# google-deepmind/meltingpot

Hardware: AMD Instinct MI355X
Metric: agent-steps/sec (env_batch x players / wall s), clean_up @4096 worlds (higher is better)
Workload: dtype u8

## Files before the change

### include/mp_engine.h

```cpp
#ifndef MP_ENGINE_H_
#define MP_ENGINE_H_

#include <stdint.h>

#ifdef __cplusplus
extern "C" {
#endif
#pragma GCC visibility push(default)

#define MP_ABI_VERSION 8

enum {
  MP_OK = 0,
  MP_ERR_INVALID = -1,
  MP_ERR_PACK = -2,
  MP_ERR_NO_DEVICE = -3,
  MP_ERR_HIP = -4,
  MP_ERR_UNSUPPORTED = -5
};

typedef enum {
  MP_EVENT_ZAP = 1,
  MP_EVENT_EDIBLE_CONSUMED = 2,
  MP_EVENT_PLAYER_CLEANED = 3,
// ... 47 lines not shown

typedef struct MpEngine MpEngine;

typedef struct {
  uint32_t struct_size;
  int32_t batch_worlds;
  int32_t waves;
  int32_t feeders;
  int32_t max_groups;
  int32_t scratch_cells;
  int32_t no_composite_cache;
  int32_t max_composites;
  int32_t verbose;
  int32_t late_feeder_prio;
  int32_t ring_batches;
  int32_t static_pct;
  int32_t world_waves;
  int32_t store_sc1;
  int32_t head;
  int32_t no_next_orders;
  int32_t record_pad;
  int32_t pace;
  int32_t team;
} MpDevOptions;

typedef struct {
  uint32_t struct_size;
  int32_t device;
  int32_t num_worlds;
  int32_t auto_reset;
  uint64_t world_offset;
  uint64_t base_seed;
  void* stream;
  int32_t num_players;
  int32_t debug_observations;
  int32_t unfused;
  int32_t literal_base_seed;
  const MpDevOptions* dev;
  const int32_t* roles;
  int32_t world_pool;
} MpConfig;

typedef struct {
  int32_t abi_version;
  int32_t substrate;
  int32_t num_worlds, num_players, num_actions;
// ... 4 lines not shown
  int32_t fused;
  int32_t num_resources;
  int32_t num_action_fields;
  int32_t plan_batch_worlds, plan_ring_batches, plan_owned_batches, plan_pooled_batches,
          plan_groups, plan_store_sc1 ;
  int32_t plan_feeders, plan_waves;
  int32_t ring_slots, ring_next;
  int32_t plan_pace, visible_layers;
  int32_t plan_team, plan_late_priority;
  int64_t retired_va_bytes, retired_va_limit;
} MpInfo;

int mp_abi_version(void);

const char* mp_last_error(void);

int mp_create(const void* pack, uint64_t pack_len, const MpConfig* cfg,
              MpEngine** out);

void mp_destroy(MpEngine* eng);

int mp_info(const MpEngine* eng, MpInfo* out);

int mp_set_stream(MpEngine* eng, void* stream);

int mp_bind_output(MpEngine* eng, MpObsKind kind, void* device_ptr);

int mp_bind_output_ring(MpEngine* eng, MpObsKind kind, void* base,
                        uint64_t slot_stride_bytes, int32_t slots);

int mp_reset(MpEngine* eng, const uint64_t* seeds, const uint8_t* mask);

int mp_step(MpEngine* eng, const int32_t* actions_device);

int mp_step_host(MpEngine* eng, const int32_t* actions_host);

int mp_step_fields(MpEngine* eng, const int32_t* fields_device);

int mp_step_fields_host(MpEngine* eng, const int32_t* fields_host);

int mp_observe(MpEngine* eng, MpObsKind kind, void* dst_device);

uint64_t mp_obs_bytes(const MpEngine* eng, MpObsKind kind);

int mp_dump(MpEngine* eng, uint8_t* grid, int32_t* avat, int32_t* glob);

// ... 76 lines not shown
```

### meltingpot_amd/_build.py

```python

from __future__ import annotations

import fcntl
import os
import shutil
import subprocess

_HERE = os.path.dirname(os.path.abspath(__file__))
CSRC = os.path.join(_HERE, "csrc")
LIB_DIR = os.path.join(_HERE, "lib")
LIB_PATH = os.path.join(LIB_DIR, "libmp_engine.so")
SOURCES = ("mp_engine.hip", "pack_decode.hip", "step_kernels.hip", "step_many.hip", "frame.hip", "frame_wpool2.hip",
           "frame_wpool4.hip", "frame_wpool8.hip")
HEADERS = ("mp_common.h", "pack_decode.h", "frame_kernel.h", "frame_wpool.h", "step_common.h", "step_clean_up.h", "step_commons.h",
           "step_territory.h", "step_coins.h", "step_matrix.h", "step_coop.h", "step_gift.h", "step_cook.h", "step_mushroom.h", "step_load.h", "../../include/mp_engine.h",
           "../../include/mp_pack.h", "exports.map")
ARCH = "gfx950"


def _stale() -> bool:
  if not os.path.exists(LIB_PATH):
    return True
  built = os.path.getmtime(LIB_PATH)
  for f in SOURCES + HEADERS:
    if os.path.getmtime(os.path.join(CSRC, f)) > built:
      return True
  return False


def build_engine(force: bool = False, verbose: bool = False) -> str:
  if not force and not _stale():
    return LIB_PATH
  hipcc = shutil.which("hipcc") or "/opt/rocm/bin/hipcc"
  if not os.path.exists(hipcc):
    raise RuntimeError("hipcc not found: cannot build libmp_engine.so")
  os.makedirs(LIB_DIR, exist_ok=True)
  with open(os.path.join(LIB_DIR, ".build.lock"), "w") as lock:
# ... 41 lines not shown
```

### meltingpot_amd/csrc/frame.hip

```cpp
#include "frame_kernel.h"

static int slot_scratch_bytes(const DevTables& t, const SubstrateTables& s) {
  int extra = 0;
  if (s.substrate == MPK_SUBSTRATE_TERRITORY) extra = stepk::extra_bytes(s.tr);
  if (s.substrate == MPK_SUBSTRATE_EXTERNALITY_MUSHROOMS) extra = stepk::extra_bytes(s.em);
  return stepk::scratch_bytes(t) + extra;
}


FramePlan plan_frame(const DevTables& t, const SubstrateTables& s, int num_worlds,
                     bool with_step, int views, int num_cus, const MpDevOptions* dev, int pool_k,
                     int world_k) {
  FramePlan p = {};
  const int lds_pool = pool_k > 1 && views != 1 ? pool_k : 0;
  const int lds_wpool = world_k > 1 && views != 0 ? world_k : 0;
  const bool world_view = views == 1;
  const int max_waves = ((with_step && s.substrate == MPK_SUBSTRATE_THE_MATRIX) ? kMatrixThreads
                                                                                : kDrawThreads) / 64;
  p.nwaves = world_view ? 12 : 16;
  p.feeders = 4;
  int B = 4, NB = 2;
  if (with_step && !world_view && max_waves == 16) {
    B = 3;
    p.feeders = s.substrate == MPK_SUBSTRATE_THE_MATRIX ? 6
// ... 217 lines not shown

template <class Tables, class Sites>
int allow_lds() {
  const void* k[9] = {
      reinterpret_cast<const void*>(&k_frame<Tables, Sites, 0>),
      reinterpret_cast<const void*>(&k_frame<Tables, Sites, 1>),
      reinterpret_cast<const void*>(&k_frame<Tables, Sites, 2>),
      reinterpret_cast<const void*>(&k_frame<Tables, Sites, 0, 2>),
      reinterpret_cast<const void*>(&k_frame<Tables, Sites, 2, 2>),
      reinterpret_cast<const void*>(&k_frame<Tables, Sites, 0, 4>),
      reinterpret_cast<const void*>(&k_frame<Tables, Sites, 2, 4>),
      reinterpret_cast<const void*>(&k_frame<Tables, Sites, 0, 8>),
      reinterpret_cast<const void*>(&k_frame<Tables, Sites, 2, 8>)};
  hipError_t r[9];
  for (int i = 0; i < 9; ++i)
    r[i] = hipFuncSetAttribute(k[i], hipFuncAttributeMaxDynamicSharedMemorySize, 160 * 1024);
  for (hipError_t e : r)
    if (e != hipSuccess) return (int)e;
  return 0;
}

}

int prepare_frame() {
  int rc = prepare_frame_wpool<2>();
  if (!rc) rc = prepare_frame_wpool<4>();
  if (!rc) rc = prepare_frame_wpool<8>();
  if (!rc) rc = allow_lds<NoTables, NoSites>();
  if (!rc) rc = allow_lds<CleanUpTables, stepk::CleanUpSites>();
#if !defined(MP_FRAME_ISA_SUBSET)
  if (!rc) rc = allow_lds<CommonsTables, stepk::CommonsSites>();
  if (!rc) rc = allow_lds<TerritoryTables, stepk::TerritorySites>();
  if (!rc) rc = allow_lds<CoinsTables, stepk::CoinsSites>();
  if (!rc) rc = allow_lds<MatrixTables, stepk::MatrixSites>();
  if (!rc) rc = allow_lds<CoopTables, stepk::CoopSites>();
  if (!rc) rc = allow_lds<GiftTables, stepk::GiftSites>();
  if (!rc) rc = allow_lds<CookTables, stepk::CookSites>();
  if (!rc) rc = allow_lds<MushroomTables, stepk::MushroomSites>();
#endif
  return rc;
}

void launch_frame(const DevTables& t, const SubstrateTables* s, const stepk::StepArgs& args,
                  uint8_t* out_a, uint8_t* out_w, const FramePlan& p, hipStream_t stream, int pool_k,
                  int world_k) {
  if (out_w && world_k > 1) {
    if (world_k == 2) launch_frame_wpool<2>(t, s, args, out_a, out_w, p, stream, pool_k);
    else if (world_k == 4) launch_frame_wpool<4>(t, s, args, out_a, out_w, p, stream, pool_k);
    else launch_frame_wpool<8>(t, s, args, out_a, out_w, p, stream, pool_k);
    return;
  }
  if (!s) {
    launch_one<NoTables, NoSites>(t, NoTables(), args, out_a, out_w, p, stream, pool_k);
    return;
  }
#if defined(MP_FRAME_ISA_SUBSET)
  if (s->substrate == MPK_SUBSTRATE_CLEAN_UP)
    launch_one<CleanUpTables, stepk::CleanUpSites>(t, s->cu, args, out_a, out_w, p, stream, pool_k);
#else
  switch (s->substrate) {
    case MPK_SUBSTRATE_CLEAN_UP:
      launch_one<CleanUpTables, stepk::CleanUpSites>(t, s->cu, args, out_a, out_w, p, stream, pool_k);
      break;
    case MPK_SUBSTRATE_COMMONS_HARVEST:
      launch_one<CommonsTables, stepk::CommonsSites>(t, s->ch, args, out_a, out_w, p, stream, pool_k);
      break;
    case MPK_SUBSTRATE_TERRITORY:
      launch_one<TerritoryTables, stepk::TerritorySites>(t, s->tr, args, out_a, out_w, p, stream, pool_k);
      break;
    case MPK_SUBSTRATE_COINS:
      launch_one<CoinsTables, stepk::CoinsSites>(t, s->co, args, out_a, out_w, p, stream, pool_k);
      break;
    case MPK_SUBSTRATE_THE_MATRIX:
      launch_one<MatrixTables, stepk::MatrixSites>(t, s->mx, args, out_a, out_w, p, stream, pool_k);
      break;
    case MPK_SUBSTRATE_COOP_MINING:
      launch_one<CoopTables, stepk::CoopSites>(t, s->cm, args, out_a, out_w, p, stream, pool_k);
      break;
// ... 13 lines not shown
```

### meltingpot_amd/csrc/frame_kernel.h

```cpp
#pragma once
#include <stdlib.h>
#include <string.h>

#include <type_traits>

#include "../../include/mp_pack.h"
#include "step_clean_up.h"
#include "step_coins.h"
#include "step_commons.h"
#include "step_coop.h"
#include "step_gift.h"
#include "step_mushroom.h"
#include "step_cook.h"
#include "step_matrix.h"
#include "step_territory.h"
#include "step_load.h"

template <bool kStep> constexpr bool nt_stores() { return kStep; }

namespace {

constexpr int kMaxLayers = 12;
constexpr int kSpriteStride = 272;
constexpr int kHeadBytes = 64;
// ... 321 lines not shown
constexpr uint64_t kMaxWaitTicks = 200000000ull;
enum { FAULT_BUFFER_FREE = 1, FAULT_BATCH_READY = 2, FAULT_PROLOGUE = 3, FAULT_CLAIM = 4 };
__device__ inline bool waited_too_long(uint32_t polls, uint64_t& t0) {
  if ((polls & 255u) != 255u) return false;
  const uint64_t now = wall_clock64();
  if (t0 == 0) { t0 = now; return false; }
  return now - t0 > kMaxWaitTicks;
}
__device__ inline void report_stall(const DevTables& t, int lane, uint32_t site, uint32_t wave,
                                    uint32_t batch, uint32_t seen, uint32_t wanted) {
  (void)lane;
  if (atomicCAS(&t.fault[0], 0u, site) == 0u) {
    t.fault[1] = blockIdx.x; t.fault[2] = wave; t.fault[3] = batch;
    t.fault[4] = seen; t.fault[5] = wanted;
  }
}

template <int kPool, int kWPool>
__device__ inline int pool_scratch_bytes(const DevTables& t) {
  if constexpr (kWPool == 0) return wave_scratch_bytes(t, kPool);
  else return wave_scratch_bytes(t, kPool, kWPool);
}

template <class Tables, class Sites, int kViews, int kPool = 0, int kWPool = 0>
__global__ __launch_bounds__(max_threads<Tables>()) void k_frame(DevTables t, Tables c,
                                                       stepk::StepArgs args,
                                                       uint8_t* __restrict__ out_a,
                                                       uint8_t* __restrict__ out_w,
                                                       FrameConsts K) {
  constexpr bool kStep = !std::is_same<Tables, NoTables>::value;
  constexpr bool kNt = nt_stores<kStep>();
#if defined(MP_FRAME_TIMELINE)
  const uint64_t tl_entry = wall_clock64();
#endif
  {
    constexpr int kArgBytes = (int)(sizeof(DevTables) + sizeof(Tables) + sizeof(stepk::StepArgs) +
                                    2 * sizeof(uint8_t*) + sizeof(FrameConsts));
    typedef const uint32_t __attribute__((address_space(4))) KernargWord;
    KernargWord* ka = (KernargWord*)__builtin_amdgcn_kernarg_segment_ptr();
    uint32_t warm = 0;
#pragma unroll
    for (int i = 0; i < kArgBytes / 4; i += 16) warm ^= ka[i];
    asm volatile("" ::"s"(warm));
  }
  extern __shared__ __attribute__((aligned(16))) uint8_t smem[];
  const FramePlan plan = K.p;
  const FrameLds lo = K.lo;
  const struct { int32_t N, nbt, chains, pool_first, b_mod_f, tables_vec, record_vec;
                 uint32_t first_k0, first_k1, magic_p, npb_all; } kc = {
      K.N, K.nbt, K.chains, K.pool_first, K.b_mod_f, K.tables_vec, K.record_vec,
      K.first_k_nibbles[0], K.first_k_nibbles[1], K.magic_p, K.npb_all};
  const int kWaves = plan.nwaves;
  const int B = plan.B, NB = plan.NB;
  const int F = plan.feeders;
// ... 995 lines not shown
```

### meltingpot_amd/csrc/mp_common.h

```cpp
#ifndef MP_COMMON_H_
#define MP_COMMON_H_

#include <hip/hip_runtime.h>
#include <stdint.h>

#include "../../include/mp_engine.h"

#define MP_MAX_PLAYERS 16
#define MP_WAVE 64

struct WorldTail {
  uint8_t ax[MP_MAX_PLAYERS];
  uint8_t ay[MP_MAX_PLAYERS];
  uint8_t aori[MP_MAX_PLAYERS];
  uint8_t aalive[MP_MAX_PLAYERS];
  uint8_t ztimer[MP_MAX_PLAYERS];
  uint8_t ctimer[MP_MAX_PLAYERS];
  uint8_t flag0[MP_MAX_PLAYERS];
  uint8_t flag1[MP_MAX_PLAYERS];
  uint8_t freeze[MP_MAX_PLAYERS];
  uint8_t removal[MP_MAX_PLAYERS];
  uint8_t aflags[MP_MAX_PLAYERS];
  uint8_t nozap[MP_MAX_PLAYERS];
  uint8_t level[MP_MAX_PLAYERS];
// ... 226 lines not shown
  int32_t n_site;
  const int32_t* site_cells;
  const int32_t* site_class;
  const int32_t* player_i32;
  const double* player_f64;
  int32_t R;
  int32_t res_layer, mark_layer, beam_layer, s_beam, hit;
  int32_t plane_a, plane_b;
  int32_t player_block;
  uint32_t s_visible_packed;
  uint64_t s_mark_packed;
  int32_t cooldown, respawn_frames, freeze, end_on_first, reset_winner, reset_loser,
      loser_dies, winner_dies, zero_inventory, random_tie, disallow_unready, has_ee,
      ee_min_frames, ee_interval, regen_delay, initial_health, n_intervals, spawn_all;
  double reward_floor, reward_multiplier, reward_unready;
  double row_matrix[9], col_matrix[9];
  double interval[10];
  uint64_t thr_regen, thr_ee;
  BeamShape shape;
};

struct SubstrateTables {
  int32_t substrate;
  CleanUpTables cu;
  CommonsTables ch;
  TerritoryTables tr;
  CoinsTables co;
  MatrixTables mx;
  CoopTables cm;
  GiftTables gr;
  CookTables cc;
  MushroomTables em;
};

struct StepOutputs {
  double* reward;
  double* ready;
  double* aux0;
  int32_t* step_type;
  double* discount;
  double* collective;
  int32_t* position;
  int32_t* orientation;
  int32_t* events;
  double* dbg[4];
  double* zap_matrix;
// ... 58 lines not shown
```

### meltingpot_amd/csrc/mp_engine.hip

```cpp
#include <chrono>
#include <map>
#include <mutex>
#include "../../include/mp_engine.h"

#include <stdarg.h>
#include <stddef.h>
#include <sys/types.h>
#include <stdio.h>
#include <string.h>

#include <algorithm>
#include <string>
#include <vector>

#include "pack_decode.h"
#include "step_common.h"

void launch_step(const DevTables& t, const SubstrateTables& s, const stepk::StepArgs& args,
                 hipStream_t stream);
void launch_step_many(const DevTables& t, const SubstrateTables& s, const stepk::StepArgs& args,
                      int steps, long long actions_step, void* const rows[5],
                      const uint64_t row_bytes[5], hipStream_t stream);
int step_lds_bytes(const DevTables& t, const SubstrateTables& s, int wpg);
int step_worlds_per_group(const DevTables& t, const SubstrateTables& s);
int prepare_step();
int prepare_step_many();
void launch_layer_view(const DevTables& t, const uint8_t* state, int32_t* out, int num_worlds,
                       hipStream_t stream);

constexpr int kFaultWords = 64 + 4 * 16 * 64 * 2;
FramePlan plan_frame(const DevTables& t, const SubstrateTables& s, int num_worlds,
                     bool with_step, int views, int num_cus, const MpDevOptions* dev,
                     int pool_k = 1,
                     int world_k = 1);
int frame_lds_bytes(const DevTables& t, const FramePlan& p, int pool_k = 1, int world_k = 1,
                    int views = 2);
int render_blob_bytes(const DevTables& t);
int prepare_frame();
// ... 719 lines not shown
    fprintf(stderr, "mp_engine: composite cache: %d images, %d table entries, probe %d\n",
            a.n_composites, a.used_slots, a.pair_probe);
  return MP_OK;
}

int upload_layer_lut(MpEngine* e) {
  const DevTables& t = e->t;
  const void* hp = e->pack.data();
  const int32_t* ssprite = table<int32_t>(hp, "state_sprite");
  const int32_t* vmap = table<int32_t>(hp, "view_sprite_map");
  std::vector<int32_t> lut((size_t)t.P * kLayerLutRow, 0);
  for (int p = 0; p < t.P; ++p) {
    const int32_t* remap = vmap + (size_t)p * t.nsprites;
    int32_t* row = lut.data() + (size_t)p * kLayerLutRow;
    for (int s = 1; s < t.nstates && s < 256; ++s)
      row[s] = ssprite[s] >= 0 ? 1 + remap[ssprite[s]] : 0;
    row[256] = 1 + remap[0];
  }
  HIP_TRY(hipMalloc((void**)&e->d_layer_lut, lut.size() * 4));
  HIP_TRY(hipMemcpy(e->d_layer_lut, lut.data(), lut.size() * 4, hipMemcpyHostToDevice));
  return MP_OK;
}

int plan_views(MpEngine* e, const MpDevOptions* dev) {
  const DevTables& t = e->t;
  for (int v = 0; v < 6; ++v) {
    FramePlan& pl = e->plan[v & 1][v >> 1];
    pl = plan_frame(t, e->sub, e->N, (v & 1) != 0, v >> 1, e->num_cus, dev);
    if (frame_lds_bytes(t, pl) > 160 * 1024)
      return fail(MP_ERR_PACK, "mp_create: renderer needs %d B of LDS", frame_lds_bytes(t, pl));
  }
  if (e->world_pool > 1)
    for (int v = 2; v < 6; ++v) {
      FramePlan& pl = e->plan[v & 1][v >> 1];
      pl = plan_frame(t, e->sub, e->N, (v & 1) != 0, v >> 1, e->num_cus, dev, 1, e->world_pool);
      const int need = frame_lds_bytes(t, pl, 1, e->world_pool, v >> 1);
      if (need > 160 * 1024)
        return fail(MP_ERR_UNSUPPORTED, "mp_create: WORLD.RGB pooled by %d (MpConfig.world_pool) needs "
                    "%d B of LDS", e->world_pool, need);
    }
  for (int i = 0; i < 3; ++i) {
    const int k = 2 << i;
    e->pool_ok[i] = t.sprite_size == 8;
    for (int v = 0; v < 6 && e->pool_ok[i]; ++v) {
      if ((v >> 1) == 1) continue;
      FramePlan& pl = e->pool_plan[i][v & 1][v >> 1];
// ... 18 lines not shown
              (v >> 1) == 0 ? "agents view" : (v >> 1) == 1 ? "world view" : "both views",
              pl.NB, pl.B, pl.feeders, pl.nwaves, pl.world_waves, pl.groups, pl.ks, pl.pool,
              frame_lds_bytes(t, pl, 1, e->world_pool, v >> 1));
    }
  return MP_OK;
}

int create_on_device(MpEngine* e, const MpConfig& cfg, DecodedPack* d) {
  const MpDevOptions* dev = cfg.dev;
  e->has_dev = dev != nullptr;
  e->next_orders = !(dev && dev->no_next_orders);
  e->device = cfg.device;
  e->N = cfg.num_worlds;
  e->auto_reset = cfg.auto_reset;
  e->stream = (hipStream_t)cfg.stream;
  e->unfused = cfg.unfused;
  e->world_pool = cfg.world_pool > 1 ? cfg.world_pool : 1;
  int cus = 0;
  if (hipDeviceGetAttribute(&cus, hipDeviceAttributeMultiprocessorCount, cfg.device) != hipSuccess ||
      cus <= 0)
    return fail(MP_ERR_NO_DEVICE, "mp_create: device %d does not report its compute units", cfg.device);
  e->num_cus = cus;
  int rc;
  if ((rc = upload_pack(e, cfg, d)) || (rc = alloc_fault_words(e)) || (rc = init_state(e, cfg)) ||
      (rc = alloc_outputs(e, cfg)) || (rc = build_atlas(e, dev, *d)) || (rc = upload_layer_lut(e)))
    return rc;
  return plan_views(e, dev);
}

}

extern "C" {

int mp_abi_version(void) { return MP_ABI_VERSION; }

const char* mp_last_error(void) { return g_error.c_str(); }

uint64_t mp_obs_bytes(const MpEngine* e, MpObsKind kind) {
  if (!e) return 0;
  const uint64_t N = (uint64_t)e->N, P = (uint64_t)e->t.P, S = (uint64_t)e->t.sprite_size;
  switch (kind) {
    case MP_OBS_RGB:
      return N * P * (e->t.vf + e->t.vb + 1) * S * (e->t.vl + e->t.vr + 1) * S * 3;
    case MP_OBS_WORLD_RGB: {
      const uint64_t k = (uint64_t)e->world_pool;
      return N * (e->t.H * S / k) * (e->t.W * S / k) * 3;
    }
    case MP_OBS_RGB_POOL2: case MP_OBS_RGB_POOL4: case MP_OBS_RGB_POOL8: {
      const uint64_t k = (uint64_t)MpEngine::pool_of(kind);
      if (!e->pool_ok[MpEngine::pool_index((int)k)]) return 0;
// ... 8 lines not shown
    case MP_OBS_AUX1: case MP_OBS_AUX2: case MP_OBS_AUX3: case MP_OBS_AUX4:
      return e->substrate == MPK_SUBSTRATE_CLEAN_UP ? N * P * 8 : 0;
    case MP_OBS_ZAP_MATRIX:
      return (e->substrate == MPK_SUBSTRATE_CLEAN_UP ||
              e->substrate == MPK_SUBSTRATE_COMMONS_HARVEST) ? N * P * P * 8 : 0;
    case MP_OBS_LAYER:
      return N * P * (e->t.vf + e->t.vb + 1) * (e->t.vl + e->t.vr + 1) * e->t.L * 4;
    case MP_OBS_INVENTORY:
      return N * P * e->inventory_types() * 8;
    case MP_OBS_INTERACTION_INVENTORIES:
      return e->substrate == MPK_SUBSTRATE_THE_MATRIX ? N * P * 2 * e->sub.mx.R * 8 : 0;
    case MP_OBS_MATRIX_CUMULANTS:
      return e->substrate == MPK_SUBSTRATE_THE_MATRIX ? N * P * (1 + 3 * e->sub.mx.R) * 8 : 0;
    case MP_OBS_INTERACTION_REWARDS:
      return e->substrate == MPK_SUBSTRATE_THE_MATRIX ? N * P * 2 * 8 : 0;
    default: return 0;
  }
}

int mp_create(const void* pack, uint64_t pack_len, const MpConfig* cfg,
              MpEngine** out) {
  if (!out) return fail(MP_ERR_INVALID, "mp_create: out is NULL");
  *out = nullptr;
  if (!cfg || (cfg->struct_size != sizeof(MpConfig) && cfg->struct_size != offsetof(MpConfig, world_pool)))
    return fail(MP_ERR_INVALID, "mp_create: bad MpConfig (struct_size)");
  MpConfig cfg_copy = {};
  memcpy(&cfg_copy, cfg, cfg->struct_size);
  if (cfg->struct_size < sizeof(MpConfig)) cfg_copy.world_pool = 1;
  cfg = &cfg_copy;
  if (cfg->dev && cfg->dev->struct_size != sizeof(MpDevOptions))
    return fail(MP_ERR_INVALID, "mp_create: bad MpDevOptions (struct_size)");
  if (cfg->num_worlds <= 0)
    return fail(MP_ERR_INVALID, "mp_create: num_worlds must be positive");
  if (cfg->unfused < 0 || cfg->unfused > 2)
    return fail(MP_ERR_INVALID, "mp_create: MpConfig.unfused must be 0, 1 or 2 (got %d)", cfg->unfused);
  if (cfg->world_pool != 0 && cfg->world_pool != 1 && cfg->world_pool != 2 && cfg->world_pool != 4 &&
      cfg->world_pool != 8)
    return fail(MP_ERR_INVALID, "mp_create: MpConfig.world_pool must be 0, 1, 2, 4 or 8 (got %d)",
                cfg->world_pool);
  const int32_t* hdr = nullptr;
  if (int rc = check_header(pack, pack_len, *cfg, &hdr)) return rc;
  std::vector<uint8_t> copy((const uint8_t*)pack, (const uint8_t*)pack + pack_len);
  if (int rc = apply_roles(copy, *cfg)) return rc;
  DecodedPack d;
  if (int rc = decode_pack(copy, *cfg, copy.data(), &d)) return rc;
  if (cfg->world_pool > 1 && d.t.sprite_size != 8)
    return fail(MP_ERR_UNSUPPORTED, "mp_create: MpConfig.world_pool needs 8 x 8 sprites (the pack's are %d x %d)",
                d.t.sprite_size, d.t.sprite_size);

  int ndev = 0;
  if (hipGetDeviceCount(&ndev) != hipSuccess || ndev <= 0)
    return fail(MP_ERR_NO_DEVICE,
                "mp_create: no HIP device; the engine has no CPU path");
  if (cfg->device < 0 || cfg->device >= ndev)
    return fail(MP_ERR_INVALID, "mp_create: device %d out of range (%d devices)",
                cfg->device, ndev);
  HIP_TRY(hipSetDevice(cfg->device));

  MpEngine* e = new MpEngine();
  e->pack = std::move(copy);
  const int rc = create_on_device(e, *cfg, &d);
  if (rc != MP_OK) {
    mp_destroy(e);
    return rc;
  }
  e->fingerprint = state_fingerprint(e->pack, e->t);
  *out = e;
  return MP_OK;
}

void mp_destroy(MpEngine* e) {
// ... 394 lines not shown
                  "that holds one step's rows of %llu bytes", kName[i], (unsigned long long)r->per_step_bytes[i],
                  (unsigned long long)elem[i], (unsigned long long)block[i]);
    if ((uintptr_t)r->per_step[i] % elem[i])
      return fail(MP_ERR_INVALID, "MpStepMany: the %s buffer %p is not %llu-byte aligned", kName[i],
                  r->per_step[i], (unsigned long long)elem[i]);
  }
  HIP_TRY(hipSetDevice(e->device));
  if (int rc = check_bank(e, r->actions, (K - 1) * r->actions_step_bytes + ablock, "MpStepMany (actions)"))
    return rc;
  for (int i = 0; i < 5; ++i) {
    if (!r->per_step[i]) continue;
    char who[48];
    snprintf(who, sizeof who, "MpStepMany (%s)", kName[i]);
    if (int rc = check_bank(e, r->per_step[i], (K - 1) * r->per_step_bytes[i] + block[i], who)) return rc;
  }
  e->touched = true;
  return submit(e, r->fields ? STEP_MODE_FIELDS : STEP_MODE_STEP, r->actions, nullptr, nullptr, nullptr, 0, r);
}

uint64_t mp_snapshot_bytes(const MpEngine* e) {
  return e ? (uint64_t)e->N * e->t.world_stride : 0;
}

int mp_snapshot(MpEngine* e, void* buf, uint64_t bytes) {
  if (e && buf && bytes == sizeof(MpWorldStates)) return world_states(e, (MpWorldStates*)buf, false);
  if (!e || !buf || bytes != mp_snapshot_bytes(e))
    return fail(MP_ERR_INVALID, "mp_snapshot: bad buffer");
  HIP_TRY(hipSetDevice(e->device));
  if (int rc = sync_and_check(e, "mp_snapshot")) return rc;
  HIP_TRY(hipMemcpy(buf, e->d_state, bytes, hipMemcpyDeviceToHost));
  return MP_OK;
}

int mp_restore(MpEngine* e, const void* buf, uint64_t bytes) {
  if (e && buf && bytes == sizeof(MpWorldStates)) {
    MpWorldStates r;
    memcpy(&r, buf, sizeof r);
    return world_states(e, &r, true);
  }
  if (buf && bytes == sizeof(MpStepMany)) {
    MpStepMany r;
    memcpy(&r, buf, sizeof r);
    return step_many(e, &r);
  }
  if (!e || !buf || bytes != mp_snapshot_bytes(e))
    return fail(MP_ERR_INVALID, "mp_restore: bad buffer");
  HIP_TRY(hipSetDevice(e->device));
// ... 703 lines not shown
```

### meltingpot_amd/engine.py

```python

from __future__ import annotations

import ctypes
import os
from typing import Dict, Optional, Sequence

import numpy as np

from meltingpot_amd import _build

OBS_RGB = 0
OBS_WORLD_RGB = 1
OBS_REWARD = 2
OBS_READY_TO_SHOOT = 3
OBS_AUX0 = 4
OBS_STEP_TYPE = 5
OBS_DISCOUNT = 6
OBS_COLLECTIVE_REWARD = 7
OBS_POSITION = 8
OBS_ORIENTATION = 9
OBS_EVENTS = 10
OBS_AUX1 = 11
OBS_AUX2 = 12
OBS_AUX3 = 13
# ... 53 lines not shown
    19: ("cooked_food_collected_from_pot", ("player_index", "cooked_item")),
}
COOKING_ITEMS = ("empty", "tomato", "dish", "soup")
MUSHROOM_TYPES = ("fullInternalityZeroExternality", "halfInternalityHalfExternality",
                  "zeroInternalityFullExternality", "negativeInternalityNegativeExternality")

COUNTER_NAMES = ("world_steps", "agent_steps", "episodes", "reward_sum_x1024",
                 "zaps", "aux0", "respawns", "bad_actions")

MP_ERR_INVALID = -1
MP_ERR_NO_DEVICE = -3
MP_ABI_VERSION = 8

ABI_SYMBOLS = (
    "mp_abi_version", "mp_last_error", "mp_create", "mp_destroy", "mp_info",
    "mp_set_stream", "mp_bind_output", "mp_reset", "mp_step", "mp_step_host",
    "mp_step_fields", "mp_step_fields_host",
    "mp_observe", "mp_obs_bytes", "mp_dump", "mp_snapshot_bytes",
    "mp_snapshot", "mp_restore", "mp_counters", "mp_sync", "mp_fault_words",
    "mp_alloc_output", "mp_free_output", "mp_tune", "mp_place_output",
    "mp_bind_output_ring", "mp_set_retired_va_limit",
    "mp_torch_alloc", "mp_torch_free", "mp_box_fill")


class MpDevOptions(ctypes.Structure):
  _fields_ = [("struct_size", ctypes.c_uint32)] + [(n, ctypes.c_int32) for n in (
      "batch_worlds", "waves", "feeders", "max_groups", "scratch_cells",
      "no_composite_cache", "max_composites", "verbose", "late_feeder_prio",
      "ring_batches", "static_pct", "world_waves", "store_sc1", "head", "no_next_orders",
      "record_pad", "pace", "team")]


class MpConfig(ctypes.Structure):
  _fields_ = [
      ("struct_size", ctypes.c_uint32),
      ("device", ctypes.c_int32),
      ("num_worlds", ctypes.c_int32),
      ("auto_reset", ctypes.c_int32),
      ("world_offset", ctypes.c_uint64),
      ("base_seed", ctypes.c_uint64),
      ("stream", ctypes.c_void_p),
      ("num_players", ctypes.c_int32),
      ("debug_observations", ctypes.c_int32),
      ("unfused", ctypes.c_int32),
      ("literal_base_seed", ctypes.c_int32),
      ("dev", ctypes.POINTER(MpDevOptions)),
      ("roles", ctypes.POINTER(ctypes.c_int32)),
      ("world_pool", ctypes.c_int32),
  ]


class MpInfo(ctypes.Structure):
  _fields_ = [(n, ctypes.c_int32) for n in (
      "abi_version", "substrate", "num_worlds", "num_players", "num_actions",
      "map_h", "map_w", "num_layers", "sprite_size", "view_h", "view_w",
      "max_frames", "world_state_bytes", "fused", "num_resources",
      "num_action_fields", "plan_batch_worlds", "plan_ring_batches", "plan_owned_batches",
      "plan_pooled_batches", "plan_groups", "plan_store_sc1", "plan_feeders", "plan_waves",
      "ring_slots", "ring_next", "plan_pace", "visible_layers", "plan_team", "plan_late_priority")] + [("retired_va_bytes", ctypes.c_int64),
                                      ("retired_va_limit", ctypes.c_int64)]


class MpPlacement(ctypes.Structure):
  _fields_ = [("candidates", ctypes.c_int32), ("picked", ctypes.c_int32),
              ("us", ctypes.c_float * 32), ("stepped", ctypes.c_int32),
              ("requested", ctypes.c_int32), ("out_of_memory", ctypes.c_int32),
              ("early_exit", ctypes.c_int32), ("setup_ms", ctypes.c_float)]


class MpBoxFill(ctypes.Structure):
  _fields_ = [("bytes", ctypes.c_uint64), ("memset_us", ctypes.c_float),
              ("product_order_us", ctypes.c_float), ("front_4k_us", ctypes.c_float),
              ("groups", ctypes.c_int32), ("waves", ctypes.c_int32), ("span_bytes", ctypes.c_uint32)]


MP_STATES_FINGERPRINT, MP_STATES_SAVE, MP_STATES_LOAD = 1, 2, 3


class MpWorldStates(ctypes.Structure):
  _fields_ = [("struct_size", ctypes.c_uint32), ("op", ctypes.c_int32),
              ("fingerprint", ctypes.c_uint64), ("worlds", ctypes.c_void_p),
              ("src", ctypes.c_void_p), ("bank", ctypes.c_void_p), ("bank_bytes", ctypes.c_uint64),
              ("count", ctypes.c_int32), ("bank_rows", ctypes.c_int32)]


def world_states_request(L, handle, op: int, **fields) -> MpWorldStates:
  req = MpWorldStates(ctypes.sizeof(MpWorldStates), op)
  for k, v in fields.items():
    setattr(req, k, v)
  call = L.mp_restore if op == MP_STATES_LOAD else L.mp_snapshot
  _check(L, call(handle, ctypes.addressof(req), ctypes.sizeof(req)),
         "mp_restore (MP_STATES_LOAD)" if op == MP_STATES_LOAD else "mp_snapshot (MpWorldStates)")
  return req


STEP_MANY_MAX = 4096
STEP_MANY_KINDS = ("reward", "collective_reward", "step_type", "discount", "events")


# ... 100 lines not shown
  L.mp_restore.argtypes = [vp, vp, u64]
  L.mp_counters.restype = i32
  L.mp_counters.argtypes = [vp, vp]
  L.mp_sync.restype = i32
  L.mp_sync.argtypes = [vp]
  L.mp_alloc_output.restype = i32
  L.mp_alloc_output.argtypes = [i32, u64, u64, ctypes.POINTER(vp)]
  L.mp_free_output.restype = i32
  L.mp_free_output.argtypes = [i32, vp]
  L.mp_tune.restype = i32
  L.mp_tune.argtypes = [vp, ctypes.POINTER(ctypes.c_double)]
  L.mp_place_output.restype = i32
  L.mp_place_output.argtypes = [vp, i32, i32, u64, ctypes.POINTER(vp), ctypes.POINTER(MpPlacement)]
  L.mp_fault_words.restype = i32
  L.mp_fault_words.argtypes = [vp, vp]
  L.mp_bind_output_ring.restype = i32
  L.mp_bind_output_ring.argtypes = [vp, i32, vp, u64, i32]
  L.mp_box_fill.restype = i32
  L.mp_box_fill.argtypes = [vp, i32, i32, ctypes.POINTER(MpBoxFill)]
  L.mp_set_retired_va_limit.restype = i32
  L.mp_set_retired_va_limit.argtypes = [ctypes.c_int64]
  _lib = L
  return L


def _check(L, rc: int, what: str):
  if rc == 0:
    return
  msg = (L.mp_last_error() or b"").decode()
  if rc == MP_ERR_INVALID:
    raise ValueError(f"{what}: {msg}")
  raise EngineError(f"{what} failed ({rc}): {msg}")


class Engine:

  def __init__(self, pack_bytes: bytes, num_worlds: int, *, device: int = 0,
               auto_reset: bool = True, world_offset: int = 0,
               base_seed: int = 0, literal_seed: bool = False, num_players: int = 0,
               debug_observations: bool = False, unfused: Optional[bool] = None,
               dev: Optional[Dict[str, int]] = None,
               roles: Optional[Sequence[int]] = None, placements: int = 8,
               world_pool: int = 1):
    if (isinstance(world_pool, bool) or not isinstance(world_pool, (int, np.integer)) or
        int(world_pool) not in (0, 1, 2, 4, 8)):
      raise ValueError(f"world_pool must be 1, 2, 4 or 8 (got {world_pool!r})")
# ... 67 lines not shown
        OBS_INVENTORY: ((self.N, self.P, info.num_resources), torch.float64),
        OBS_INTERACTION_INVENTORIES: ((self.N, self.P, 2, info.num_resources), torch.float64),
        OBS_MATRIX_CUMULANTS: ((self.N, self.P, 1 + 3 * info.num_resources), torch.float64),
        OBS_INTERACTION_REWARDS: ((self.N, self.P, 2), torch.float64),
        **{kind: ((self.N, self.P, info.view_h * S // k, info.view_w * S // k, 3), torch.uint8)
           for k, kind in OBS_RGB_POOL.items()},
    }
    self._bound: Dict[int, "torch.Tensor"] = {}

  @property
  def fused(self) -> bool:
    info = MpInfo()
    _check(self._L, self._L.mp_info(self._h, ctypes.byref(info)), "mp_info")
    return bool(info.fused)

  @property
  def plan(self) -> Dict[str, int]:
    info = MpInfo()
    _check(self._L, self._L.mp_info(self._h, ctypes.byref(info)), "mp_info")
    return {"batch_worlds": info.plan_batch_worlds, "ring_batches": info.plan_ring_batches,
            "owned_batches": info.plan_owned_batches, "pooled_batches": info.plan_pooled_batches,
            "workgroups": info.plan_groups, "sc1_stores": info.plan_store_sc1,
            "feeders": info.plan_feeders, "waves": info.plan_waves, "pace": info.plan_pace,
            "xcd_teams": info.plan_team, "late_feeder_priority": info.plan_late_priority}

  def close(self):
    if getattr(self, "_h", None):
      self._L.mp_destroy(self._h)
      self._h = None
      self._bound.clear()

  def __del__(self):
    try:
      self.close()
    except Exception:
      pass

  def __enter__(self):
    return self

  def __exit__(self, *exc):
    self.close()

  def events(self, world: int = 0):
    return self.events_all(worlds=[world])[0]

  def events_all(self, worlds=None):
# ... 418 lines not shown
```

Baseline: 293.8 million.

## Add constant-specialized clean_up frame kernel selected by pack hash

Adds a stock kernel variant that pins all DevTables and CleanUpTables fields to compile-time constants for the standard clean_up pack. The variant is selected at create time when the pack hash and decoded fields match, with an option to force the generic kernel. The intent is to let the compiler fold map sizes, layer indices and thresholds, cutting address arithmetic, table loads and register pressure. The cost is extra code size and a kernel that only applies to one exact configuration.

Measured after the change: 319.4 million, median of 6. +8.7%, better.

```diff
diff --git a/include/mp_engine.h b/include/mp_engine.h
--- a/include/mp_engine.h
+++ b/include/mp_engine.h
@@ -93,6 +93,7 @@
   int32_t record_pad;
   int32_t pace;
   int32_t team;
+  int32_t generic_kernel;
 } MpDevOptions;
 
 typedef struct {
@@ -143,6 +144,17 @@
 
 int mp_info(const MpEngine* eng, MpInfo* out);
 
+enum { MP_KERNEL_GENERIC = 0, MP_KERNEL_STOCK = 1 };
+typedef struct {
+  uint32_t struct_size;
+  int32_t variant;
+  const void* pack;
+  uint64_t pack_len;
+  const MpConfig* cfg;
+  char* fields;
+  uint64_t fields_cap;
+} MpKernelVariant;
+
 int mp_set_stream(MpEngine* eng, void* stream);
 
 int mp_bind_output(MpEngine* eng, MpObsKind kind, void* device_ptr);
diff --git a/include/mp_kernel_variant.h b/include/mp_kernel_variant.h
--- /dev/null
+++ b/include/mp_kernel_variant.h
@@ -0,0 +1,23 @@
+#ifndef MP_KERNEL_VARIANT_H_
+#define MP_KERNEL_VARIANT_H_
+
+#include <string.h>
+
+#include "mp_engine.h"
+
+static inline int mp_kernel_variant(MpEngine* eng, const void* pack, uint64_t pack_len,
+                                    const MpConfig* cfg, char* fields, uint64_t fields_cap) {
+  MpKernelVariant r;
+  int rc;
+  memset(&r, 0, sizeof r);
+  r.struct_size = sizeof r;
+  r.pack = pack;
+  r.pack_len = pack_len;
+  r.cfg = cfg;
+  r.fields = fields;
+  r.fields_cap = fields_cap;
+  rc = mp_snapshot(eng, &r, sizeof r);
+  return rc != MP_OK ? rc : r.variant;
+}
+
+#endif
diff --git a/meltingpot_amd/_build.py b/meltingpot_amd/_build.py
--- a/meltingpot_amd/_build.py
+++ b/meltingpot_amd/_build.py
@@ -11,8 +11,8 @@
 LIB_DIR = os.path.join(_HERE, "lib")
 LIB_PATH = os.path.join(LIB_DIR, "libmp_engine.so")
 SOURCES = ("mp_engine.hip", "pack_decode.hip", "step_kernels.hip", "step_many.hip", "frame.hip", "frame_wpool2.hip",
-           "frame_wpool4.hip", "frame_wpool8.hip")
-HEADERS = ("mp_common.h", "pack_decode.h", "frame_kernel.h", "frame_wpool.h", "step_common.h", "step_clean_up.h", "step_commons.h",
+           "frame_wpool4.hip", "frame_wpool8.hip", "frame_stock.hip")
+HEADERS = ("mp_common.h", "stock.h", "stock_clean_up.h", "pack_decode.h", "frame_kernel.h", "frame_wpool.h", "step_common.h", "step_clean_up.h", "step_commons.h",
            "step_territory.h", "step_coins.h", "step_matrix.h", "step_coop.h", "step_gift.h", "step_cook.h", "step_mushroom.h", "step_load.h", "../../include/mp_engine.h",
            "../../include/mp_pack.h", "exports.map")
 ARCH = "gfx950"
diff --git a/meltingpot_amd/csrc/frame.hip b/meltingpot_amd/csrc/frame.hip
--- a/meltingpot_amd/csrc/frame.hip
+++ b/meltingpot_amd/csrc/frame.hip
@@ -263,8 +263,13 @@
 
 }
 
+int prepare_frame_stock();
+void launch_frame_stock(const DevTables& t, const CleanUpTables& c, const stepk::StepArgs& args,
+                        uint8_t* out_a, uint8_t* out_w, const FramePlan& p, hipStream_t stream);
+
 int prepare_frame() {
   int rc = prepare_frame_wpool<2>();
+  if (!rc) rc = prepare_frame_stock();
   if (!rc) rc = prepare_frame_wpool<4>();
   if (!rc) rc = prepare_frame_wpool<8>();
   if (!rc) rc = allow_lds<NoTables, NoSites>();
@@ -295,6 +300,10 @@
     launch_one<NoTables, NoSites>(t, NoTables(), args, out_a, out_w, p, stream, pool_k);
     return;
   }
+  if (s->stock == MP_KERNEL_STOCK && s->substrate == MPK_SUBSTRATE_CLEAN_UP && !(out_a && pool_k > 1)) {
+    launch_frame_stock(t, s->cu, args, out_a, out_w, p, stream);
+    return;
+  }
 #if defined(MP_FRAME_ISA_SUBSET)
   if (s->substrate == MPK_SUBSTRATE_CLEAN_UP)
     launch_one<CleanUpTables, stepk::CleanUpSites>(t, s->cu, args, out_a, out_w, p, stream, pool_k);
diff --git a/meltingpot_amd/csrc/frame_kernel.h b/meltingpot_amd/csrc/frame_kernel.h
--- a/meltingpot_amd/csrc/frame_kernel.h
+++ b/meltingpot_amd/csrc/frame_kernel.h
@@ -367,7 +367,11 @@
   else return wave_scratch_bytes(t, kPool, kWPool);
 }
 
-template <class Tables, class Sites, int kViews, int kPool = 0, int kWPool = 0>
+struct NoStock {
+  template <class Tables>
+  __device__ static inline void pin(DevTables&, Tables&) {}
+};
+template <class Tables, class Sites, int kViews, int kPool = 0, int kWPool = 0, class Stock = NoStock>
 __global__ __launch_bounds__(max_threads<Tables>()) void k_frame(DevTables t, Tables c,
                                                        stepk::StepArgs args,
                                                        uint8_t* __restrict__ out_a,
@@ -375,6 +379,7 @@
                                                        FrameConsts K) {
   constexpr bool kStep = !std::is_same<Tables, NoTables>::value;
   constexpr bool kNt = nt_stores<kStep>();
+  Stock::pin(t, c);
 #if defined(MP_FRAME_TIMELINE)
   const uint64_t tl_entry = wall_clock64();
 #endif
diff --git a/meltingpot_amd/csrc/frame_stock.hip b/meltingpot_amd/csrc/frame_stock.hip
--- /dev/null
+++ b/meltingpot_amd/csrc/frame_stock.hip
@@ -0,0 +1,42 @@
+#include "frame_kernel.h"
+#include "stock.h"
+
+namespace {
+
+template <int kViews>
+void launch_stock(const DevTables& t, const CleanUpTables& c, const stepk::StepArgs& args,
+                  uint8_t* out_a, uint8_t* out_w, const FrameConsts& K, const FramePlan& p,
+                  hipStream_t stream) {
+  hipLaunchKernelGGL((k_frame<CleanUpTables, stepk::CleanUpSites, kViews, 0, 0, StockCleanUp>),
+                     dim3(p.groups), dim3(p.nwaves * 64), (size_t)K.lo.total, stream, t, c, args,
+                     out_a, out_w, K);
+}
+
+}
+
+int prepare_frame_stock() {
+  const void* k[3] = {
+      reinterpret_cast<const void*>(&k_frame<CleanUpTables, stepk::CleanUpSites, 0, 0, 0, StockCleanUp>),
+      reinterpret_cast<const void*>(&k_frame<CleanUpTables, stepk::CleanUpSites, 1, 0, 0, StockCleanUp>),
+      reinterpret_cast<const void*>(&k_frame<CleanUpTables, stepk::CleanUpSites, 2, 0, 0, StockCleanUp>)};
+  for (const void* f : k) {
+    const hipError_t e = hipFuncSetAttribute(f, hipFuncAttributeMaxDynamicSharedMemorySize, 160 * 1024);
+    if (e != hipSuccess) return (int)e;
+  }
+  return 0;
+}
+
+void launch_frame_stock(const DevTables& t, const CleanUpTables& c, const stepk::StepArgs& args,
+                        uint8_t* out_a, uint8_t* out_w, const FramePlan& p, hipStream_t stream) {
+  FrameConsts K = frame_consts(t, p, args.num_worlds, true, 0);
+  if (out_a && out_w) {
+    K.npb_all = K.npb[0] + K.npb[1];
+    launch_stock<2>(t, c, args, out_a, out_w, K, p, stream);
+  } else if (out_w) {
+    K.npb_all = K.npb[1];
+    launch_stock<1>(t, c, args, out_a, out_w, K, p, stream);
+  } else {
+    K.npb_all = K.npb[0];
+    launch_stock<0>(t, c, args, out_a, out_w, K, p, stream);
+  }
+}
diff --git a/meltingpot_amd/csrc/mp_common.h b/meltingpot_amd/csrc/mp_common.h
--- a/meltingpot_amd/csrc/mp_common.h
+++ b/meltingpot_amd/csrc/mp_common.h
@@ -272,6 +272,7 @@
 
 struct SubstrateTables {
   int32_t substrate;
+  int32_t stock;
   CleanUpTables cu;
   CommonsTables ch;
   TerritoryTables tr;
diff --git a/meltingpot_amd/csrc/mp_engine.hip b/meltingpot_amd/csrc/mp_engine.hip
--- a/meltingpot_amd/csrc/mp_engine.hip
+++ b/meltingpot_amd/csrc/mp_engine.hip
@@ -14,6 +14,7 @@
 #include <vector>
 
 #include "pack_decode.h"
+#include "stock.h"
 #include "step_common.h"
 
 void launch_step(const DevTables& t, const SubstrateTables& s, const stepk::StepArgs& args,
@@ -779,6 +780,20 @@
   return MP_OK;
 }
 
+uint64_t pack_hash(const std::vector<uint8_t>& pack) {
+  uint64_t h = 0xcbf29ce484222325ull;
+  for (uint8_t b : pack) { h ^= b; h *= 0x100000001b3ull; }
+  return h;
+}
+
+int select_kernels(const std::vector<uint8_t>& pack, const DecodedPack& d, const MpDevOptions* dev) {
+  if (dev && dev->generic_kernel) return MP_KERNEL_GENERIC;
+  if (d.sub.substrate == MPK_SUBSTRATE_CLEAN_UP && pack_hash(pack) == MP_STOCK_CLEAN_UP_PACK_HASH &&
+      StockCleanUp::matches(d.t, d.sub.cu))
+    return MP_KERNEL_STOCK;
+  return MP_KERNEL_GENERIC;
+}
+
 int plan_views(MpEngine* e, const MpDevOptions* dev) {
   const DevTables& t = e->t;
   for (int v = 0; v < 6; ++v) {
@@ -843,10 +858,65 @@
     return fail(MP_ERR_NO_DEVICE, "mp_create: device %d does not report its compute units", cfg.device);
   e->num_cus = cus;
   int rc;
-  if ((rc = upload_pack(e, cfg, d)) || (rc = alloc_fault_words(e)) || (rc = init_state(e, cfg)) ||
+  if ((rc = upload_pack(e, cfg, d))) return rc;
+  e->sub.stock = select_kernels(e->pack, *d, dev);
+  if ((rc = alloc_fault_words(e)) || (rc = init_state(e, cfg)) ||
       (rc = alloc_outputs(e, cfg)) || (rc = build_atlas(e, dev, *d)) || (rc = upload_layer_lut(e)))
     return rc;
   return plan_views(e, dev);
+}
+
+struct HostStage {
+  MpConfig cfg = {};
+  MpDevOptions dev = {};
+  std::vector<uint8_t> pack;
+  DecodedPack d;
+};
+
+int host_stage(const void* pack, uint64_t pack_len, const MpConfig* cfg, HostStage* h) {
+  if (!cfg || (cfg->struct_size != sizeof(MpConfig) && cfg->struct_size != offsetof(MpConfig, world_pool)))
+    return fail(MP_ERR_INVALID, "mp_create: bad MpConfig (struct_size)");
+  memcpy(&h->cfg, cfg, cfg->struct_size);
+  if (cfg->struct_size < sizeof(MpConfig)) h->cfg.world_pool = 1;
+  cfg = &h->cfg;
+  if (cfg->dev) {
+    if (cfg->dev->struct_size != sizeof(MpDevOptions) &&
+        cfg->dev->struct_size != offsetof(MpDevOptions, generic_kernel))
+      return fail(MP_ERR_INVALID, "mp_create: bad MpDevOptions (struct_size)");
+    memcpy(&h->dev, cfg->dev, cfg->dev->struct_size);
+    h->dev.struct_size = sizeof(MpDevOptions);
+    h->cfg.dev = &h->dev;
+  }
+  if (cfg->num_worlds <= 0)
+    return fail(MP_ERR_INVALID, "mp_create: num_worlds must be positive");
+  if (cfg->unfused < 0 || cfg->unfused > 2)
+    return fail(MP_ERR_INVALID, "mp_create: MpConfig.unfused must be 0, 1 or 2 (got %d)", cfg->unfused);
+  if (cfg->world_pool != 0 && cfg->world_pool != 1 && cfg->world_pool != 2 && cfg->world_pool != 4 &&
+      cfg->world_pool != 8)
+    return fail(MP_ERR_INVALID, "mp_create: MpConfig.world_pool must be 0, 1, 2, 4 or 8 (got %d)",
+                cfg->world_pool);
+  const int32_t* hdr = nullptr;
+  if (int rc = check_header(pack, pack_len, *cfg, &hdr)) return rc;
+  h->pack.assign((const uint8_t*)pack, (const uint8_t*)pack + pack_len);
+  if (int rc = apply_roles(h->pack, *cfg)) return rc;
+  if (int rc = decode_pack(h->pack, *cfg, h->pack.data(), &h->d)) return rc;
+  if (cfg->world_pool > 1 && h->d.t.sprite_size != 8)
+    return fail(MP_ERR_UNSUPPORTED, "mp_create: MpConfig.world_pool needs 8 x 8 sprites (the pack's are %d x %d)",
+                h->d.t.sprite_size, h->d.t.sprite_size);
+  return MP_OK;
+}
+
+void literal(std::string* out, int32_t v) { *out += std::to_string(v); }
+void literal(std::string* out, uint32_t v) { *out += std::to_string(v) + "u"; }
+void literal(std::string* out, uint64_t v) {
+  char b[32];
+  snprintf(b, sizeof b, "0x%llxull", (unsigned long long)v);
+  *out += b;
+}
+void literal(std::string* out, double v) {
+  char b[48];
+  snprintf(b, sizeof b, "%a", v);
+  *out += b;
 }
 
 }
@@ -901,31 +971,11 @@
               MpEngine** out) {
   if (!out) return fail(MP_ERR_INVALID, "mp_create: out is NULL");
   *out = nullptr;
-  if (!cfg || (cfg->struct_size != sizeof(MpConfig) && cfg->struct_size != offsetof(MpConfig, world_pool)))
-    return fail(MP_ERR_INVALID, "mp_create: bad MpConfig (struct_size)");
-  MpConfig cfg_copy = {};
-  memcpy(&cfg_copy, cfg, cfg->struct_size);
-  if (cfg->struct_size < sizeof(MpConfig)) cfg_copy.world_pool = 1;
-  cfg = &cfg_copy;
-  if (cfg->dev && cfg->dev->struct_size != sizeof(MpDevOptions))
-    return fail(MP_ERR_INVALID, "mp_create: bad MpDevOptions (struct_size)");
-  if (cfg->num_worlds <= 0)
-    return fail(MP_ERR_INVALID, "mp_create: num_worlds must be positive");
-  if (cfg->unfused < 0 || cfg->unfused > 2)
-    return fail(MP_ERR_INVALID, "mp_create: MpConfig.unfused must be 0, 1 or 2 (got %d)", cfg->unfused);
-  if (cfg->world_pool != 0 && cfg->world_pool != 1 && cfg->world_pool != 2 && cfg->world_pool != 4 &&
-      cfg->world_pool != 8)
-    return fail(MP_ERR_INVALID, "mp_create: MpConfig.world_pool must be 0, 1, 2, 4 or 8 (got %d)",
-                cfg->world_pool);
-  const int32_t* hdr = nullptr;
-  if (int rc = check_header(pack, pack_len, *cfg, &hdr)) return rc;
-  std::vector<uint8_t> copy((const uint8_t*)pack, (const uint8_t*)pack + pack_len);
-  if (int rc = apply_roles(copy, *cfg)) return rc;
-  DecodedPack d;
-  if (int rc = decode_pack(copy, *cfg, copy.data(), &d)) return rc;
-  if (cfg->world_pool > 1 && d.t.sprite_size != 8)
-    return fail(MP_ERR_UNSUPPORTED, "mp_create: MpConfig.world_pool needs 8 x 8 sprites (the pack's are %d x %d)",
-                d.t.sprite_size, d.t.sprite_size);
+  HostStage h;
+  if (int rc = host_stage(pack, pack_len, cfg, &h)) return rc;
+  cfg = &h.cfg;
+  std::vector<uint8_t>& copy = h.pack;
+  DecodedPack& d = h.d;
 
   int ndev = 0;
   if (hipGetDeviceCount(&ndev) != hipSuccess || ndev <= 0)
@@ -1366,7 +1416,39 @@
   return e ? (uint64_t)e->N * e->t.world_stride : 0;
 }
 
+static_assert(sizeof(MpKernelVariant) != sizeof(MpWorldStates) && sizeof(MpKernelVariant) != sizeof(MpStepMany),
+              "mp_snapshot / mp_restore tell their requests apart by size");
+static int kernel_variant(const MpEngine* e, MpKernelVariant* r) {
+  if (r->struct_size != sizeof(MpKernelVariant))
+    return fail(MP_ERR_INVALID, "MpKernelVariant: struct_size %u, expected %zu", r->struct_size, sizeof(MpKernelVariant));
+  if (e) { r->variant = e->sub.stock; return MP_OK; }
+  char* fields = r->fields;
+  const uint64_t fields_cap = r->fields_cap;
+  HostStage h;
+  if (int rc = host_stage(r->pack, r->pack_len, r->cfg, &h)) return rc;
+  if (fields) {
+    if (h.d.sub.substrate != MPK_SUBSTRATE_CLEAN_UP)
+      return fail(MP_ERR_UNSUPPORTED, "MpKernelVariant: no stock kernels for this level");
+    std::string text;
+#define MP_FIELD_T(f) text += "t " #f " "; literal(&text, h.d.t.f); text += "\n";
+#define MP_FIELD_C(f) text += "c " #f " "; literal(&text, h.d.sub.cu.f); text += "\n";
+    MP_STOCK_DEV_FIELDS(MP_FIELD_T)
+    MP_STOCK_CLEAN_UP_FIELDS(MP_FIELD_C)
+#undef MP_FIELD_T
+#undef MP_FIELD_C
+    text += "hash ";
+    literal(&text, pack_hash(h.pack));
+    text += "\n";
+    if (text.size() + 1 > fields_cap)
+      return fail(MP_ERR_INVALID, "MpKernelVariant: fields needs %zu bytes", text.size() + 1);
+    memcpy(fields, text.c_str(), text.size() + 1);
+  }
+  r->variant = select_kernels(h.pack, h.d, h.cfg.dev);
+  return MP_OK;
+}
+
 int mp_snapshot(MpEngine* e, void* buf, uint64_t bytes) {
+  if (buf && bytes == sizeof(MpKernelVariant)) return kernel_variant(e, (MpKernelVariant*)buf);
   if (e && buf && bytes == sizeof(MpWorldStates)) return world_states(e, (MpWorldStates*)buf, false);
   if (!e || !buf || bytes != mp_snapshot_bytes(e))
     return fail(MP_ERR_INVALID, "mp_snapshot: bad buffer");
diff --git a/meltingpot_amd/csrc/stock.h b/meltingpot_amd/csrc/stock.h
--- /dev/null
+++ b/meltingpot_amd/csrc/stock.h
@@ -0,0 +1,45 @@
+#ifndef MP_STOCK_H_
+#define MP_STOCK_H_
+
+#include "mp_common.h"
+#include "stock_clean_up.h"
+
+#define MP_STOCK_DEV_FIELDS(X)                                                                   \
+  X(H) X(W) X(L) X(P) X(nstates) X(nsprites) X(topology) X(max_frames) X(nact) X(nfields)       \
+  X(field_lo) X(field_hi) X(P_pack) X(avatar_layer) X(sprite_size) X(vl) X(vr) X(vf) X(vb)      \
+  X(grid_planes) X(grid_bytes) X(grid_pad) X(world_stride) X(n_spawn) X(n_init_groups)          \
+  X(n_optional) X(optional_spawn)
+
+#define MP_STOCK_CLEAN_UP_FIELDS(X)                                                              \
+  X(n_apple) X(n_dirt) X(n_water) X(thr_dirt_spawn) X(thr_episode_end)                          \
+  X(s_apple) X(s_apple_wait) X(s_dirt) X(s_dirt_wait)                                           \
+  X(s_water[0]) X(s_water[1]) X(s_water[2]) X(s_water[3]) X(s_water_packed)                     \
+  X(apple_layer) X(dirt_layer) X(dirt_wait_layer) X(water_layer)                                \
+  X(clean_layer) X(s_clean_hit) X(clean_hit) X(clean_cooldown) X(clean_length) X(clean_radius)  \
+  X(dirt_delay) X(ee_min_frames) X(ee_interval) X(anim_frames) X(n_dirt_init) X(eat_reward)     \
+  X(zap.cooldown) X(zap.length) X(zap.radius) X(zap.respawn_frames) X(zap.remove_hit)           \
+  X(zap.layer) X(zap.s_hit) X(zap.hit) X(zap.penalty) X(zap.reward)                             \
+  X(zap.shape.n) X(zap.shape.per) X(zap.shape.magic)                                            \
+  X(clean_shape.n) X(clean_shape.per) X(clean_shape.magic)
+
+struct StockCleanUp {
+  __host__ __device__ static inline void pin(DevTables& t, CleanUpTables& c) {
+#define MP_STOCK_PIN_T(f, v) t.f = v;
+#define MP_STOCK_PIN_C(f, v) c.f = v;
+    MP_STOCK_CLEAN_UP_T(MP_STOCK_PIN_T)
+    MP_STOCK_CLEAN_UP_C(MP_STOCK_PIN_C)
+#undef MP_STOCK_PIN_T
+#undef MP_STOCK_PIN_C
+  }
+  static inline bool matches(const DevTables& t, const CleanUpTables& c) {
+#define MP_STOCK_SAME_T(f, v) if (!(t.f == v)) return false;
+#define MP_STOCK_SAME_C(f, v) if (!(c.f == v)) return false;
+    MP_STOCK_CLEAN_UP_T(MP_STOCK_SAME_T)
+    MP_STOCK_CLEAN_UP_C(MP_STOCK_SAME_C)
+#undef MP_STOCK_SAME_T
+#undef MP_STOCK_SAME_C
+    return true;
+  }
+};
+
+#endif
diff --git a/meltingpot_amd/csrc/stock_clean_up.h b/meltingpot_amd/csrc/stock_clean_up.h
--- /dev/null
+++ b/meltingpot_amd/csrc/stock_clean_up.h
@@ -0,0 +1,77 @@
+#pragma once
+#define MP_STOCK_CLEAN_UP_PACK_HASH 0x647be3be5e193cb8ull
+#define MP_STOCK_CLEAN_UP_T(X) \
+  X(H, 21) \
+  X(W, 30) \
+  X(L, 9) \
+  X(P, 7) \
+  X(nstates, 50) \
+  X(nsprites, 33) \
+  X(topology, 0) \
+  X(max_frames, 5000) \
+  X(nact, 9) \
+  X(nfields, 4) \
+  X(field_lo, 65280u) \
+  X(field_hi, 16843012u) \
+  X(P_pack, 15) \
+  X(avatar_layer, 6) \
+  X(sprite_size, 8) \
+  X(vl, 5) \
+  X(vr, 5) \
+  X(vf, 9) \
+  X(vb, 1) \
+  X(grid_planes, 9) \
+  X(grid_bytes, 5670) \
+  X(grid_pad, 5680) \
+  X(world_stride, 6080) \
+  X(n_spawn, 19) \
+  X(n_init_groups, 1) \
+  X(n_optional, 0) \
+  X(optional_spawn, 0)
+#define MP_STOCK_CLEAN_UP_C(X) \
+  X(n_apple, 122) \
+  X(n_dirt, 147) \
+  X(n_water, 167) \
+  X(thr_dirt_spawn, 0x10000000000000ull) \
+  X(thr_episode_end, 0x6666666666667ull) \
+  X(s_apple, 45) \
+  X(s_apple_wait, 46) \
+  X(s_dirt, 38) \
+  X(s_dirt_wait, 37) \
+  X(s_water[0], 33) \
+  X(s_water[1], 34) \
+  X(s_water[2], 35) \
+  X(s_water[3], 36) \
+  X(s_water_packed, 606282273u) \
+  X(apple_layer, 4) \
+  X(dirt_layer, 4) \
+  X(dirt_wait_layer, 0) \
+  X(water_layer, 2) \
+  X(clean_layer, 8) \
+  X(s_clean_hit, 49) \
+  X(clean_hit, 1) \
+  X(clean_cooldown, 2) \
+  X(clean_length, 3) \
+  X(clean_radius, 1) \
+  X(dirt_delay, 50) \
+  X(ee_min_frames, 1000) \
+  X(ee_interval, 100) \
+  X(anim_frames, 2) \
+  X(n_dirt_init, 79) \
+  X(eat_reward, 0x1p+0) \
+  X(zap.cooldown, 10) \
+  X(zap.length, 3) \
+  X(zap.radius, 1) \
+  X(zap.respawn_frames, 50) \
+  X(zap.remove_hit, 1) \
+  X(zap.layer, 7) \
+  X(zap.s_hit, 48) \
+  X(zap.hit, 0) \
+  X(zap.penalty, 0x0p+0) \
+  X(zap.reward, 0x0p+0) \
+  X(zap.shape.n, 9) \
+  X(zap.shape.per, 7) \
+  X(zap.shape.magic, 7282u) \
+  X(clean_shape.n, 9) \
+  X(clean_shape.per, 7) \
+  X(clean_shape.magic, 7282u)
diff --git a/meltingpot_amd/engine.py b/meltingpot_amd/engine.py
--- a/meltingpot_amd/engine.py
+++ b/meltingpot_amd/engine.py
@@ -99,13 +99,15 @@
     "mp_bind_output_ring", "mp_set_retired_va_limit",
     "mp_torch_alloc", "mp_torch_free", "mp_box_fill")
 
+KERNEL_GENERIC, KERNEL_STOCK = 0, 1
+
 
 class MpDevOptions(ctypes.Structure):
   _fields_ = [("struct_size", ctypes.c_uint32)] + [(n, ctypes.c_int32) for n in (
       "batch_worlds", "waves", "feeders", "max_groups", "scratch_cells",
       "no_composite_cache", "max_composites", "verbose", "late_feeder_prio",
       "ring_batches", "static_pct", "world_waves", "store_sc1", "head", "no_next_orders",
-      "record_pad", "pace", "team")]
+      "record_pad", "pace", "team", "generic_kernel")]
 
 
 class MpConfig(ctypes.Structure):
@@ -152,6 +154,13 @@
 
 
 MP_STATES_FINGERPRINT, MP_STATES_SAVE, MP_STATES_LOAD = 1, 2, 3
+
+
+class MpKernelVariant(ctypes.Structure):
+  _fields_ = [("struct_size", ctypes.c_uint32), ("variant", ctypes.c_int32),
+              ("pack", ctypes.c_void_p), ("pack_len", ctypes.c_uint64),
+              ("cfg", ctypes.POINTER(MpConfig)), ("fields", ctypes.c_void_p),
+              ("fields_cap", ctypes.c_uint64)]
 
 
 class MpWorldStates(ctypes.Structure):
@@ -298,6 +307,29 @@
   L.mp_set_retired_va_limit.argtypes = [ctypes.c_int64]
   _lib = L
   return L
+
+
+def kernel_variant(pack_bytes: bytes, *, num_players: int = 0,
+                   dev: Optional[Dict[str, int]] = None) -> int:
+  return pack_fields(pack_bytes, num_players=num_players, dev=dev)[0]
+
+
+def pack_fields(pack_bytes: bytes, *, num_players: int = 0, dev: Optional[Dict[str, int]] = None,
+                want_fields: bool = False):
+  L = load_library()
+  cfg = MpConfig(ctypes.sizeof(MpConfig), 0, 1, 1, 0, 0, None, int(num_players))
+  if dev:
+    opts = MpDevOptions(ctypes.sizeof(MpDevOptions), max_composites=-1)
+    for k, v in dev.items():
+      setattr(opts, k, int(v))
+    cfg.dev = ctypes.pointer(opts)
+  buf = ctypes.create_string_buffer(pack_bytes, len(pack_bytes))
+  out = ctypes.create_string_buffer(1 << 16) if want_fields else None
+  req = MpKernelVariant(ctypes.sizeof(MpKernelVariant), 0, ctypes.addressof(buf), len(pack_bytes),
+                        ctypes.pointer(cfg), ctypes.addressof(out) if out else None,
+                        len(out) if out else 0)
+  _check(L, L.mp_snapshot(None, ctypes.addressof(req), ctypes.sizeof(req)), "mp_snapshot (MpKernelVariant)")
+  return req.variant, (out.value.decode() if out else "")
 
 
 def _check(L, rc: int, what: str):
@@ -411,7 +443,14 @@
             "owned_batches": info.plan_owned_batches, "pooled_batches": info.plan_pooled_batches,
             "workgroups": info.plan_groups, "sc1_stores": info.plan_store_sc1,
             "feeders": info.plan_feeders, "waves": info.plan_waves, "pace": info.plan_pace,
-            "xcd_teams": info.plan_team, "late_feeder_priority": info.plan_late_priority}
+            "xcd_teams": info.plan_team, "late_feeder_priority": info.plan_late_priority,
+            "stock": self._kernel_variant()}
+
+  def _kernel_variant(self) -> int:
+    req = MpKernelVariant(ctypes.sizeof(MpKernelVariant))
+    if self._L.mp_snapshot(self._h, ctypes.addressof(req), ctypes.sizeof(req)) != 0:
+      return KERNEL_GENERIC
+    return int(req.variant)
 
   def close(self):
     if getattr(self, "_h", None):
```
